# DRSY/EasyKV

Hardware: AMD Instinct MI355X
Metric: decode_tokens_per_sec (higher is better)
Workload: dtype f16 storage / f32 accumulate; 1 GPU; bench-D decode at fixed budget: B=1 L=32 Hq=32 H=32 D=128 budget=2048 T=2049 kv_policy=roco (Llama2-7B shape, budget=50% of S=4096); parallelism=1 GPU, layers_per_launch=32, layers_per_rank=32, sequences_per_launch=1, n_split=1, fused=True, slot_map=scattered (random permutation: long-run steady state), prewarm_steps=4096, hipgraph=False, overlap_scorer=False, handoff=False

## Files before the change

### easykv_amd/csrc/ekv_attn_decode.inc

```
#ifdef EKV_TAIL_PROFILE
#define EKV_STAMP(i) do { if (threadIdx.x == 0) stamps[i] = __builtin_readcyclecounter(); } while (0)
#endif
#include "ekv_decode_stream.h"
#include "ekv_decode_tail.h"
#ifndef EKV_KV8
#define EKV_KV8 0
#endif
#ifndef EKV_BATCH
#define EKV_BATCH 0
#endif
#if EKV_BATCH && EKV_KV8
#error "batch instances: 16-bit rows, plain keys"
#endif
#define ekv_attn_decode_kernel EKV_KERNEL_NAME(ekv_attn_decode_kernel)
#define ekv_decode_fused_kernel EKV_KERNEL_NAME(ekv_decode_fused_kernel)
#ifndef EKV_SPLIT_KU
#define EKV_SPLIT_KU (EKV_KV8 ? 4 : 8)
#endif
#ifndef EKV_FUSED_KU
#define EKV_FUSED_KU (EKV_KV8 ? 4 : 8)
#endif
#ifndef EKV_ROPE_KU
#define EKV_ROPE_KU(rep) ((rep) == 4 ? 8 : 4)
#endif

namespace {

constexpr int kEPL = EKV_KV8 ? 16 : 8;

template <int D, int REP, bool ROPE, bool SLOT_LDS>
__global__ void __launch_bounds__(256) ekv_attn_decode_kernel(const EkvAttnArgs EKV_ARG_A EKV_TB_PARAM) {
  EKV_SHADOW_A(blockIdx.z)
  using Gm = EkvDecodeGeom<D>;
  extern __shared__ __attribute__((aligned(16))) char smem[];
  int32_t* s_slot = reinterpret_cast<int32_t*>(smem);
  float* s_part = reinterpret_cast<float*>(smem + (SLOT_LDS ? ekv_align((size_t)a.rows_per_split * 4, 16) : 0));

  const int split = blockIdx.x % a.n_split, qgrp = blockIdx.x / a.n_split, h = blockIdx.y, ll = blockIdx.z;
  const int rep_all = a.n_q_heads / a.n_kv_heads;
  const int hq0 = h * rep_all + qgrp * REP;
  const int nrep = (REP == 1 || REP == 2) ? REP : min(REP, rep_all - qgrp * REP);
  const int tid = threadIdx.x;
  const int t0 = split * a.rows_per_split;
  const int t1 = min(a.n_slots, t0 + a.rows_per_split);
  const size_t head_row = ((size_t)(a.layer_begin + ll) * a.n_kv_heads + h) * a.cap;
  if (SLOT_LDS) {
    for (int i = tid; i < t1 - t0; i += 256) s_slot[i] = a.slot_of_pos[head_row + t0 + i];
    __syncthreads();
  }

  float m[REP], l[REP], o[REP][kEPL];
  float* logits = a.logits ? a.logits + ((size_t)ll * a.n_q_heads + hq0) * a.t_pad : nullptr;
  constexpr int KU = (!ROPE && !SLOT_LDS && REP <= 2) ? EKV_SPLIT_KU : (EKV_KV8 ? 4 : 8);
  ekv_decode_stream<D, REP, ROPE, SLOT_LDS, 4, false, KU>(a, SLOT_LDS ? s_slot : a.slot_of_pos + head_row, logits, a.t_pad, t0, t1,
                                                          ll, h, head_row, m, l, o, nullptr, EkvNoop(), nrep, hq0);

  ekv_decode_wave_combine<D, REP>(m, l, o);
  ekv_decode_stash<D, REP>(s_part, m, l, o);
  __syncthreads();
  const bool fold_here = a.arrive != nullptr;
  for (int idx = tid; idx < REP * D; idx += 256) {
    const int r = idx / D, d = idx % D;
    if (r >= nrep) continue;
    float mm, ls, os;
    ekv_decode_reduce<D, REP>(s_part, r, d, mm, ls, os);
    float* dst = a.partials + (((size_t)ll * a.n_q_heads + hq0 + r) * a.n_split + split) * Gm::PS;
    if (fold_here) {
      if (d == 0) {
        ekv_store_sc1(dst, mm);
        ekv_store_sc1(dst + 1, ls);
      }
      ekv_store_sc1(dst + 2 + d, os);
    } else {
      if (d == 0) {
        dst[0] = mm;
        dst[1] = ls;
      }
      dst[2 + d] = os;
    }
  }
  if (!fold_here) return;
  asm volatile("s_waitcnt vmcnt(0)" ::: "memory");
  __syncthreads();
  uint32_t* s_last = reinterpret_cast<uint32_t*>(s_part);
  if (tid == 0) {
    uint32_t* word = a.arrive + (size_t)EKV_ARRIVE_ROW(ll) * a.n_kv_heads + h;
    const uint32_t old = __hip_atomic_fetch_add(word, 1u, __ATOMIC_RELAXED, __HIP_MEMORY_SCOPE_AGENT);
    const bool last = (int)(old + 1u) == a.n_split;
    if (last) __hip_atomic_store(word, 0u, __ATOMIC_RELAXED, __HIP_MEMORY_SCOPE_AGENT);
    *s_last = last ? 1u : 0u;
  }
  __syncthreads();
  if (*s_last == 0u) return;
  const __amdgpu_buffer_rsrc_t rsrc = __builtin_amdgcn_make_buffer_rsrc(
      a.partials + (size_t)ll * a.n_q_heads * a.n_split * Gm::PS, 0, (int)((size_t)a.n_q_heads * a.n_split * Gm::PS * 4), 0x00020000);
  for (int idx = tid; idx < nrep * D; idx += 256) {
    const int r = idx / D, d = idx % D;
    const size_t row = (size_t)ll * a.n_q_heads + hq0 + r;
    a.out_direct[row * D + d] = ekv_to_e(ekv_fold_partials_buf_auto(rsrc, (unsigned)((hq0 + r) * a.n_split * Gm::PS), a.n_split, Gm::PS, d));
  }
}

template <int D, int REP, bool ROPE, int ITEMS, int NW, bool SLOT>
__global__ void __launch_bounds__(64 * NW, (NW >= 8 ? (REP == 1 ? 2 : 1) : (SLOT && ITEMS > 12 ? 2 : (REP == 1 ? 4 : (REP == 2 ? 3 : 2))))) ekv_decode_fused_kernel(const EkvAttnArgs EKV_ARG_A, const EkvScoreArgs EKV_ARG_SC EKV_TB_PARAM) {
  EKV_SHADOW_A(blockIdx.z)
  EKV_SHADOW_SC(blockIdx.z)
  using Gm = EkvDecodeGeom<D, NW>;
  extern __shared__ __attribute__((aligned(16))) char smem[];
  const int h = blockIdx.y, ll = blockIdx.z, tid = threadIdx.x;
  const int lane = tid & 63, wave = tid >> 6;
  const int T = a.n_slots;
  const int nrep = (REP == 1 || REP == 2) ? REP : a.n_q_heads / a.n_kv_heads;
  const bool roco = sc.policy == EKV_POLICY_ROCO;
  const bool scored = roco || sc.policy == EKV_POLICY_H2O_HEAD || sc.policy == EKV_POLICY_TOVA;
  const int off = scored ? sc.score_off : 0;
  const int W = SLOT ? a.phys_extent : T - off;
  const int w_pad = (int)ekv_align((size_t)W, 256);
#ifdef EKV_NO_PHYS
  constexpr bool PHYS = false;
#else
  constexpr bool PHYS = !ROPE;
#endif
  const int l_pad = a.l_pad;
  float* s_logit = reinterpret_cast<float*>(smem);
  float* s_part = s_logit + (size_t)REP * l_pad;
  float* sS = s_part + (size_t)Gm::NP * REP * Gm::PS + ((Gm::NP * REP * Gm::PS) & 3 ? 4 - ((Gm::NP * REP * Gm::PS) & 3) : 0);
  float* sQ = sS + w_pad;
  float* sC = sQ + w_pad;
  RedN<NW> red;
  red.buf = reinterpret_cast<unsigned long long*>(sS + (size_t)(roco ? (SLOT ? 2 : 3) : 1) * w_pad);
  red.phase = 0;
  red.lane = lane;
  red.wave = wave;
  const size_t head_row = ((size_t)(a.layer_begin + ll) * a.n_kv_heads + h) * a.cap;
#ifdef EKV_TAIL_PROFILE
  unsigned long long* stamps = reinterpret_cast<unsigned long long*>(sc.tova_row) + ((size_t)ll * a.n_kv_heads + h) * 8;
#endif
  EKV_STAMP(0);
  constexpr bool kOrders = D == 128 && REP == 1 && !ROPE && NW == 4 && SLOT && ITEMS <= 12 && !EKV_KV8 && !EKV_BATCH;
  bool order_k = false;
  if constexpr (kOrders) {
    const int om = a.fused_order & 3;
    if (om == 2) {
      order_k = scored;
    } else if (om == 1 && scored) {
      uint32_t* s_flag = reinterpret_cast<uint32_t*>(red.buf);
      if (tid == 0) {
        const uint32_t hw = __builtin_amdgcn_s_getreg(63492);
        const int src = (a.fused_order >> 4) & 3;
        const uint32_t x = src == 0 ? (hw >> 16) & 15u : (src == 1 ? hw & 15u : (uint32_t)(ll * a.n_kv_heads + h));
        const bool below = (x & ((a.fused_order >> 8) & 15u)) < ((a.fused_order >> 12) & 15u);
        *s_flag = below != (((a.fused_order >> 6) & 1) != 0) ? 1u : 0u;
      }
      __syncthreads();
      order_k = __builtin_amdgcn_readfirstlane((int)*s_flag) != 0;
    }
  }
  const int32_t* slot_row = a.slot_of_pos + head_row;
  uint32_t* s_deadw = reinterpret_cast<uint32_t*>(red.buf + 2 * NW * 8);
  if (scored) ekv_tail_prefetch_rows<NW, false>(sc, head_row, W, w_pad, roco, sS, sQ, sC, !SLOT);
  float g_old = 0.f, c_new = 0.f;
  int nb = 0;
  if (SLOT) {
    const size_t head = (size_t)(a.layer_begin + ll) * a.n_kv_heads + h;
    g_old = sc.slot_state[4 * head];
    nb = reinterpret_cast<const int32_t*>(sc.slot_state)[4 * head + 1];
    c_new = sc.cnt_tail[head_row + T - 1] - g_old;
  }
  const int E = a.phys_extent;
  const int fl_idx = T - 1 + tid;
  int fl = 0;
  if (PHYS) {
    fl = slot_row[min(fl_idx, a.cap - 1)];
    const int n_words = (int)ekv_align((size_t)E, 128) / 32;
    for (int i = tid; i < n_words; i += 64 * NW)
      s_deadw[i] = i * 32 >= E ? ~0u : (i * 32 + 32 > E ? ~0u << (E & 31) : 0u);
  }
  auto mask_ready = [&]() {
    ekv_lds_barrier();
    if (fl_idx < a.cap && fl < E) atomicOr(&s_deadw[fl >> 5], 1u << (fl & 31));
    for (int i = fl_idx + 64 * NW; i < a.cap; i += 64 * NW) {
      const int row = slot_row[i];
      if (row < E) atomicOr(&s_deadw[row >> 5], 1u << (row & 31));
    }
    ekv_lds_barrier();
  };

  if constexpr (kOrders) {
    if (order_k) {
      constexpr int LPR = Gm::LPR;
      const int sub = lane % LPR, grp = lane / LPR;
      const int new_row = slot_row[T - 1];
      const uint8_t* s_dead = reinterpret_cast<const uint8_t*>(s_deadw);
      const uint4 qv = reinterpret_cast<const uint4*>(a.q + ((size_t)ll * a.n_q_heads + h) * D)[sub];
      float mk = EKV_NEG_INF;
      ekv_decode_plane_loop<D, NW>(a.k, head_row, E, mask_ready, [&](uint4 (&kr)[8], const int j0) {
        const unsigned dead8 = (unsigned)s_dead[j0 >> 3];
        float s[8];
#pragma unroll
        for (int u = 0; u < 8; ++u) {
          const float acc = ekv_group_sum<LPR>(ekv_dot8(qv, kr[u], 0.f));
          s[u] = !((dead8 >> u) & 1u) ? acc / a.sm_div : EKV_NEG_INF;
        }
        float mine = s[0];
#pragma unroll
        for (int u = 1; u < 8; ++u) mine = (sub == u) ? s[u] : mine;
        if (sub < 8 && !((dead8 >> sub) & 1u)) s_logit[j0 + sub] = mine;
#pragma unroll
        for (int u = 0; u < 8; ++u) mk = fmaxf(mk, s[u]);
      });
      const __half* v_new_row = a.v_new + ((size_t)ll * a.n_kv_heads + h) * D;
      if (wave == 0 && grp == 0) {
        const uint4 kn = reinterpret_cast<const uint4*>(a.k_new + ((size_t)ll * a.n_kv_heads + h) * D)[sub];
        const uint4 vn = reinterpret_cast<const uint4*>(v_new_row)[sub];
        const size_t off_new = (head_row + new_row) * D;
        reinterpret_cast<uint4*>(a.k_w + off_new)[sub] = kn;
        reinterpret_cast<uint4*>(a.v_w + off_new)[sub] = vn;
        const float acc = ekv_group_sum<LPR>(ekv_dot8(qv, kn, 0.f)) / a.sm_div;
        if (sub == 0) s_logit[new_row] = acc;
        mk = fmaxf(mk, acc);
      }
      ekv_tail_prefetch_ragged<NW>(sc, head_row, W, roco, sS, sQ, sC, false);
      float cC[ITEMS];
      int32_t cB[ITEMS];
#pragma unroll
      for (int it = 0; it < ITEMS; ++it) {
        const int j = min(tid + it * 64 * NW, a.cap - 1);
        cC[it] = roco ? sc.score_cnt[head_row + j] : 0.f;
        cB[it] = sc.birth[head_row + j];
      }
      EKV_STAMP(1);
      mk = ekv_wave_max(mk);
      if (lane == 0) s_part[(size_t)wave * Gm::PS] = mk;
      __syncthreads();
      uint32_t* s_hist = s_deadw + ekv_align(ekv_align((size_t)l_pad, 128) / 32, 4);
      ekv_decode_tail_slot<REP, ITEMS, NW, true>(sc, ll, h, head_row, T, E, s_logit, l_pad, sS, sQ, cC, cB, red, s_hist,
                                                 reinterpret_cast<unsigned long long*>(s_part), Gm::NP * REP * Gm::PS / 2, s_part, Gm::NP,
                                                 Gm::PS, s_deadw, new_row, g_old, c_new, nb, nrep);
      EKV_STAMP(2);
      float m[1] = {EKV_NEG_INF}, l[1] = {0.f}, o[1][8];
#pragma unroll
      for (int i = 0; i < 8; ++i) o[0][i] = 0.f;
      ekv_decode_plane_loop<D, NW>(a.v, head_row, E, EkvNoop(), [&](uint4 (&vr)[8], const int j0) {
        const unsigned dead8 = (unsigned)s_dead[j0 >> 3];
        float s[8];
        if (dead8 == 0xFFu) {
#pragma unroll
          for (int u = 0; u < 8; ++u) s[u] = EKV_NEG_INF;
        } else {
          const float4 s0 = *reinterpret_cast<const float4*>(s_logit + j0), s1 = *reinterpret_cast<const float4*>(s_logit + j0 + 4);
          s[0] = s0.x, s[1] = s0.y, s[2] = s0.z, s[3] = s0.w, s[4] = s1.x, s[5] = s1.y, s[6] = s1.z, s[7] = s1.w;
        }
        if (dead8 != 0u) {
#pragma unroll
          for (int u = 0; u < 8; ++u)
            if ((dead8 >> u) & 1u) {
              vr[u] = uint4{0, 0, 0, 0};
              s[u] = EKV_NEG_INF;
            }
        }
        float mx = s[0];
#pragma unroll
        for (int u = 1; u < 8; ++u) mx = fmaxf(mx, s[u]);
        const float mn = fmaxf(m[0], mx);
        if (mn == EKV_NEG_INF) return;
        const float alpha = exp2f((m[0] - mn) * EKV_LOG2E);
        l[0] *= alpha;
#pragma unroll
        for (int i = 0; i < 8; ++i) o[0][i] *= alpha;
#pragma unroll
        for (int u = 0; u < 8; ++u) {
          const float p = exp2f((s[u] - mn) * EKV_LOG2E);
          l[0] += p;
          ekv_axpy8(p, vr[u], o[0]);
        }
        m[0] = mn;
      });
      if (wave == 0 && grp == 0) {
        const uint4 vn = reinterpret_cast<const uint4*>(v_new_row)[sub];
        const float acc = s_logit[new_row];
        const float mn = fmaxf(m[0], acc);
        const float alpha = m[0] == EKV_NEG_INF ? 0.f : exp2f((m[0] - mn) * EKV_LOG2E);
        const float p = exp2f((acc - mn) * EKV_LOG2E);
        l[0] = l[0] * alpha + p;
#pragma unroll
        for (int i = 0; i < 8; ++i) o[0][i] *= alpha;
        ekv_axpy8(p, vn, o[0]);
        m[0] = mn;
      }
      ekv_decode_wave_combine<D, 1>(m, l, o);
      ekv_decode_stash<D, 1, NW>(s_part, m, l, o);
      __syncthreads();
      for (int d = tid; d < D; d += 64 * NW) {
        float mm, ls, os;
        ekv_decode_reduce<D, 1, NW>(s_part, 0, d, mm, ls, os);
        sc.out[((size_t)ll * a.n_q_heads + h) * D + d] = ekv_to_e(os / ls);
      }
      EKV_STAMP(5);
#ifdef EKV_TAIL_PROFILE
      if (tid == 0) {
        stamps[3] = 1;
        stamps[6] = __builtin_amdgcn_s_getreg(63492);
        stamps[7] = __builtin_amdgcn_s_getreg(63508);
      }
#endif
      return;
    }
  }

  constexpr int KUF = ROPE ? EKV_ROPE_KU(REP) : EKV_FUSED_KU;
  float m[REP], l[REP], o[REP][kEPL];
  if (PHYS)
    ekv_decode_stream<D, REP, ROPE, false, NW, PHYS, KUF>(a, slot_row, s_logit, l_pad, 0, T, ll, h, head_row, m, l, o,
                                                     reinterpret_cast<const uint8_t*>(s_deadw), mask_ready, nrep, h * nrep);
  else
    ekv_decode_stream<D, REP, ROPE, false, NW, false, KUF>(a, slot_row, s_logit, l_pad, 0, T, ll, h, head_row, m, l, o, nullptr, EkvNoop(),
                                                      nrep, h * nrep);
  if (scored) ekv_tail_prefetch_ragged<NW>(sc, head_row, W, roco, sS, sQ, sC, !SLOT);
  float cC[SLOT ? ITEMS : 1];
  int32_t cB[SLOT ? ITEMS : 1];
  if (SLOT) {
#pragma unroll
    for (int it = 0; it < (SLOT ? ITEMS : 1); ++it) {
      const int j = min(tid + it * 64 * NW, a.cap - 1);
      cC[it] = roco ? sc.score_cnt[head_row + j] : 0.f;
      cB[it] = sc.birth[head_row + j];
    }
  }

  EKV_STAMP(1);
  ekv_decode_wave_combine<D, REP>(m, l, o);
  ekv_decode_stash<D, REP, NW>(s_part, m, l, o);
  __syncthreads();
  for (int idx = tid; idx < nrep * D; idx += 64 * NW) {
    const int r = idx / D, d = idx % D;
    float mm, ls, os;
    ekv_decode_reduce<D, REP, NW>(s_part, r, d, mm, ls, os);
    sc.out[((size_t)ll * a.n_q_heads + h * nrep + r) * D + d] = ekv_to_e(os / ls);
  }

  uint32_t* s_hist = s_deadw + ekv_align(ekv_align((size_t)l_pad, 128) / 32, 4);
  if constexpr (SLOT) {
    ekv_decode_tail_slot<REP, ITEMS, NW>(sc, ll, h, head_row, T, E, s_logit, l_pad, sS, sQ, cC, cB, red, s_hist,
                                         reinterpret_cast<unsigned long long*>(s_part), Gm::NP * REP * Gm::PS / 2, s_part, Gm::NP, Gm::PS,
                                         s_deadw, slot_row[T - 1], g_old, c_new, nb, nrep);
  } else {
    ekv_decode_tail<REP, ITEMS, NW, PHYS>(sc, ll, h, head_row, T, off, W, s_logit, l_pad, sS, sQ, sC, red, s_hist,
                                          reinterpret_cast<unsigned long long*>(s_part), Gm::NP * REP * Gm::PS / 2, s_part, Gm::NP, Gm::PS, nrep);
  }
  EKV_STAMP(5);
#ifdef EKV_TAIL_PROFILE
  if (tid == 0) {
    stamps[6] = __builtin_amdgcn_s_getreg(63492);
    stamps[7] = __builtin_amdgcn_s_getreg(63508);
  }
#endif
}

template <int REP>
hipError_t launch(const EkvAttnArgs& a EKV_TB_DECL, int layer_count, hipStream_t s) {
  using Gm = EkvDecodeGeom<EKV_D>;
  const size_t part = (size_t)Gm::NP * REP * Gm::PS * 4;
  const int rep_all = a.n_q_heads / a.n_kv_heads;
  const dim3 grid(a.n_split * ((rep_all + REP - 1) / REP), a.n_kv_heads, layer_count);
  if ((a.cap & 3) == 0 && a.cap >= 16) {
    hipLaunchKernelGGL((ekv_attn_decode_kernel<EKV_D, REP, EKV_ROPE, false>), grid, dim3(256), part, s, a EKV_TB_PASS);
  } else {
    const size_t lds = ekv_align((size_t)a.rows_per_split * 4, 16) + part;
    if (lds > 48 * 1024)
      (void)hipFuncSetAttribute(reinterpret_cast<const void*>(&ekv_attn_decode_kernel<EKV_D, REP, EKV_ROPE, true>),
                                hipFuncAttributeMaxDynamicSharedMemorySize, (int)lds);
    hipLaunchKernelGGL((ekv_attn_decode_kernel<EKV_D, REP, EKV_ROPE, true>), grid, dim3(256), lds, s, a EKV_TB_PASS);
  }
  return hipGetLastError();
}

template <int REP, int NW = 8>
size_t fused_lds(int t_pad, int l_pad, int n_state) { return ekv_fused_lds<EKV_D, REP, NW>(t_pad, l_pad, n_state); }

template <int REP, int ITEMS, int NW, bool SLOT>
hipError_t launch_fused_k(const EkvAttnArgs& a, const EkvScoreArgs& sc EKV_TB_DECL, int layer_count, hipStream_t s) {
  const size_t lds = SLOT ? fused_lds<REP, NW>(a.phys_extent, a.l_pad, sc.policy == EKV_POLICY_ROCO ? 2 : 1)
                          : fused_lds<REP, NW>(a.t_pad, a.l_pad, sc.policy == EKV_POLICY_ROCO ? 3 : 1);
  if (lds > 48 * 1024)
    (void)hipFuncSetAttribute(reinterpret_cast<const void*>(&ekv_decode_fused_kernel<EKV_D, REP, EKV_ROPE, ITEMS, NW, SLOT>),
                              hipFuncAttributeMaxDynamicSharedMemorySize, (int)lds);
  hipLaunchKernelGGL((ekv_decode_fused_kernel<EKV_D, REP, EKV_ROPE, ITEMS, NW, SLOT>), dim3(1, a.n_kv_heads, layer_count),
                     dim3(64 * NW), lds, s, a, sc EKV_TB_PASS);
  return hipGetLastError();
}

template <int REP, int NW>
hipError_t launch_fused_nw(const EkvAttnArgs& a, const EkvScoreArgs& sc EKV_TB_DECL, int layer_count, hipStream_t s) {
  constexpr int NT = 64 * NW, I0 = (2304 + NT - 1) / NT, I1 = (6144 + NT - 1) / NT;
  if (sc.birth != nullptr) {
    if constexpr (!EKV_ROPE && !EKV_BATCH && REP <= 4) {
      if (a.phys_extent <= NT * I0) return launch_fused_k<REP, I0, NW, true>(a, sc EKV_TB_PASS, layer_count, s);
      if (a.phys_extent <= NT * I1) return launch_fused_k<REP, I1, NW, true>(a, sc EKV_TB_PASS, layer_count, s);
    }
    return hipErrorInvalidValue;
  }
  if (a.n_slots <= NT * I0) return launch_fused_k<REP, I0, NW, false>(a, sc EKV_TB_PASS, layer_count, s);
  return launch_fused_k<REP, I1, NW, false>(a, sc EKV_TB_PASS, layer_count, s);
}
template <int REP>
hipError_t launch_fused(const EkvAttnArgs& a, const EkvScoreArgs& sc EKV_TB_DECL, int layer_count, int nw, hipStream_t s) {
  return nw == 8 ? launch_fused_nw<REP, 8>(a, sc EKV_TB_PASS, layer_count, s) : launch_fused_nw<REP, 4>(a, sc EKV_TB_PASS, layer_count, s);
}

}

#if EKV_ROPE
#define EKV_KEYS rope
#else
#define EKV_KEYS plain
#endif
#define EKV_SYM(fn) EKV_FN_DECODE(fn, EKV_D, EKV_KEYS, EKV_ELEM, EKV_ROWS, EKV_BATCHING)

hipError_t EKV_SYM(ekv_launch_attn_decode)(const EkvAttnArgs& a, const EkvSeqTable* tb, int rep, int layer_count, hipStream_t s) {
  if (rep < 1) return hipErrorInvalidValue;
  switch (rep) {
    case 1: return launch<1>(a EKV_TB_DEREF, layer_count, s);
    case 2: return launch<2>(a EKV_TB_DEREF, layer_count, s);
    case 3: case 4: return launch<4>(a EKV_TB_DEREF, layer_count, s);
    default: return launch<8>(a EKV_TB_DEREF, layer_count, s);
  }
}

hipError_t EKV_SYM(ekv_launch_decode_fused)(const EkvAttnArgs& a, const EkvScoreArgs& sc, const EkvSeqTable* tb, int rep, int layer_count,
                                            int nw, hipStream_t s) {
  switch (rep) {
    case 1: return launch_fused<1>(a, sc EKV_TB_DEREF, layer_count, nw, s);
    case 2: return launch_fused<2>(a, sc EKV_TB_DEREF, layer_count, nw, s);
    case 3: case 4: return launch_fused<4>(a, sc EKV_TB_DEREF, layer_count, nw, s);
    case 5: case 6: case 7: case 8: return launch_fused<8>(a, sc EKV_TB_DEREF, layer_count, nw, s);
    default: return hipErrorInvalidValue;
  }
}
```

### easykv_amd/csrc/ekv_decode_stream.h

```cpp
#pragma once
#include "ekv_common.h"
#include "ekv_kernels.h"

constexpr int kU = 8;

template <int D, int NW = 4, int KU = kU, int EPL = 8>
struct EkvDecodeGeom {
  static constexpr int LIVE = D / EPL;
  static constexpr int LPR = LIVE <= 4 ? 4 : (LIVE <= 8 ? 8 : 16);
  static constexpr int G = 64 / LPR;
  static constexpr int RW = G * KU;
  static constexpr int NP = NW;
  static constexpr int PS = D + 2;
};

template <int D, int REP, int NW = 8>
inline size_t ekv_fused_lds(int t_pad, int l_pad, int n_state) {
  using Gm = EkvDecodeGeom<D, NW>;
  const size_t part = ekv_align((size_t)Gm::NP * REP * Gm::PS, 4);
  return ((size_t)REP * l_pad + part + (size_t)n_state * ekv_align((size_t)t_pad, 256)) * 4 + 2 * NW * 8 * 8 +
         ekv_align(ekv_align((size_t)l_pad, 128) / 8, 16) + 264 * 4;
}
template <int D>
inline size_t ekv_fused_lds_max(int rep, int t_pad, int l_pad, int nw) {
  switch (rep) {
    case 1: return nw == 8 ? ekv_fused_lds<D, 1, 8>(t_pad, l_pad, 3) : ekv_fused_lds<D, 1, 4>(t_pad, l_pad, 3);
    case 2: return nw == 8 ? ekv_fused_lds<D, 2, 8>(t_pad, l_pad, 3) : ekv_fused_lds<D, 2, 4>(t_pad, l_pad, 3);
    case 3: case 4: return nw == 8 ? ekv_fused_lds<D, 4, 8>(t_pad, l_pad, 3) : ekv_fused_lds<D, 4, 4>(t_pad, l_pad, 3);
    default: return nw == 8 ? ekv_fused_lds<D, 8, 8>(t_pad, l_pad, 3) : ekv_fused_lds<D, 8, 4>(t_pad, l_pad, 3);
  }
}

struct EkvNoop {
  __device__ __forceinline__ void operator()() const {}
};
#ifndef EKV_ROPE_MOCK
#define EKV_ROPE_MOCK 0
#endif
template <int D, int REP, bool ROPE, bool SLOT_LDS, int NW = 4, bool PHYS = false, int KU = kU, typename MaskReady = EkvNoop, int EPL = 8>
__device__ __forceinline__ void ekv_decode_stream(const EkvAttnArgs& a, const int32_t* s_slot, float* logit_out,
                                                  int logit_stride, int t0, int t1_in, int ll, int h, size_t head_row,
                                                  float (&m)[REP], float (&l)[REP], float (&o)[REP][EPL],
                                                  const uint8_t* s_dead = nullptr, MaskReady mask_ready = MaskReady(),
                                                  int n_rep_real = 0, int q_head0 = -1) {
  using Gm = EkvDecodeGeom<D, NW, KU, EPL>;
  constexpr int LPR = Gm::LPR, RW = Gm::RW, LIVE = Gm::LIVE;
  constexpr bool KV8 = EPL == 16;
  static_assert(EPL == 8 || (KV8 && !ROPE && LIVE == LPR), "FP8 rows: plain keys, head_dim 64 / 128");
  constexpr int ESZ = KV8 ? 1 : 2;
  constexpr bool PADDED = LIVE != LPR;
  constexpr int kNW = NW;
  static_assert(!(PHYS && (ROPE || SLOT_LDS)), "physical-order streaming: plain keys, global slot map");
  static_assert((KU == 4 || KU == 8 || KU == 16) && (!PHYS || KU <= 8), "4, 8 or 16 rows per lane group; the dead-row mask is one byte per 8 rows");
  const int tid = threadIdx.x, lane = tid & 63, wave = tid >> 6;
  const int sub = lane % LPR, grp = lane / LPR;
  const int t_new = a.n_slots - 1;
  int t1 = t1_in;
  const bool live_lane = !PADDED || sub < LIVE;
  const int nrep = n_rep_real > 0 ? n_rep_real : REP;
  const int hq0 = q_head0 >= 0 ? q_head0 : h * REP;

  uint4 qv[REP], qv1[REP];
  float qf[REP][8];
#pragma unroll
  for (int r = 0; r < REP; ++r) {
    const __half* qp = a.q + ((size_t)ll * a.n_q_heads + hq0 + min(r, nrep - 1)) * D;
    qv[r] = live_lane ? reinterpret_cast<const uint4*>(qp)[sub * (EPL / 8)] : uint4{0, 0, 0, 0};
    qv1[r] = KV8 ? reinterpret_cast<const uint4*>(qp)[sub * 2 + 1] : uint4{0, 0, 0, 0};
#pragma unroll
    for (int i = 0; i < 8; ++i) qf[r][i] = 0.f;
    if (ROPE && live_lane) {
      const int half_d = D / 2;
      const float* c = a.rope_cos + (size_t)t_new * D;
      const float* s = a.rope_sin + (size_t)t_new * D;
#pragma unroll
      for (int i = 0; i < 8; ++i) {
        const int d = sub * 8 + i;
        const int dp = d < half_d ? d + half_d : d - half_d;
        const float x = __half2float(qp[d]), y = __half2float(qp[dp]);
        qf[r][i] = x * c[d] + (d < half_d ? -y : y) * s[d];
      }
    }
  }

#ifndef EKV_ROPE_EXACT
#define EKV_ROPE_EXACT 0
#endif
  constexpr bool kRopeExact = EKV_ROPE_EXACT || REP == 8;
  const float sgn = (sub < LIVE / 2) ? -1.f : 1.f;
  const int tab_off = (sub % (LIVE / 2)) * 8;
  auto rope_seed = [&](int j, ekv_f2 (&cc)[4], ekv_f2 (&ss)[4]) {
#if EKV_ROPE_MOCK == 1
    float one = 1.f, zero = 0.25f;
    asm volatile("" : "+v"(one), "+v"(zero));
#pragma unroll
    for (int i = 0; i < 4; ++i) cc[i] = ekv_f2{one, one}, ss[i] = ekv_f2{zero, zero};
    (void)j;
#else
    const float4* c4 = reinterpret_cast<const float4*>(a.rope_cos + (size_t)j * D + tab_off);
    const float4* s4 = reinterpret_cast<const float4*>(a.rope_sin + (size_t)j * D + tab_off);
    const float4 c0 = c4[0], c1 = c4[1], s0 = s4[0], s1 = s4[1];
    cc[0] = ekv_f2{c0.x, c0.y}, cc[1] = ekv_f2{c0.z, c0.w}, cc[2] = ekv_f2{c1.x, c1.y}, cc[3] = ekv_f2{c1.z, c1.w};
    ss[0] = ekv_f2{s0.x, s0.y} * sgn, ss[1] = ekv_f2{s0.z, s0.w} * sgn, ss[2] = ekv_f2{s1.x, s1.y} * sgn, ss[3] = ekv_f2{s1.z, s1.w} * sgn;
#endif
  };
  ekv_f2 stp_c[4], stp_s[4];
  if (ROPE && !kRopeExact) rope_seed(min(1, a.n_slots - 1), stp_c, stp_s);
  auto rope_advance = [&](ekv_f2 (&cc)[4], ekv_f2 (&ss)[4]) {
#pragma unroll
    for (int i = 0; i < 4; ++i) {
      const ekv_f2 cn = __builtin_elementwise_fma(cc[i], stp_c[i], -(ss[i] * stp_s[i]));
      ss[i] = __builtin_elementwise_fma(ss[i], stp_c[i], cc[i] * stp_s[i]);
      cc[i] = cn;
    }
  };
  auto rope_rotate = [&](const uint4& kv, const ekv_f2 (&cc)[4], const ekv_f2 (&ss)[4], float (&kp)[8]) {
    uint4 other;
#if EKV_ROPE_MOCK == 2
    other = kv;
#else
    if (PADDED) {
      const int src = (lane & ~(LPR - 1)) | (sub < LIVE / 2 ? sub + LIVE / 2 : (sub < LIVE ? sub - LIVE / 2 : sub));
      other.x = __shfl(kv.x, src, 64);
      other.y = __shfl(kv.y, src, 64);
      other.z = __shfl(kv.z, src, 64);
      other.w = __shfl(kv.w, src, 64);
    } else {
      other.x = __shfl_xor(kv.x, LPR / 2, 64);
      other.y = __shfl_xor(kv.y, LPR / 2, 64);
      other.z = __shfl_xor(kv.z, LPR / 2, 64);
      other.w = __shfl_xor(kv.w, LPR / 2, 64);
    }
#endif
    const ekv_h8 kh = __builtin_bit_cast(ekv_h8, kv), oh = __builtin_bit_cast(ekv_h8, other);
#pragma unroll
    for (int i = 0; i < 4; ++i) {
      const ekv_f2 k2 = {(float)kh[2 * i], (float)kh[2 * i + 1]}, o2 = {(float)oh[2 * i], (float)oh[2 * i + 1]};
      const ekv_f2 r2 = __builtin_elementwise_fma(k2, cc[i], o2 * ss[i]);
      kp[2 * i] = r2[0];
      kp[2 * i + 1] = r2[1];
    }
  };

  const __half* k_new_row = a.k_new + ((size_t)ll * a.n_kv_heads + h) * D;
  const __half* v_new_row = a.v_new + ((size_t)ll * a.n_kv_heads + h) * D;
  const int slot_base = SLOT_LDS ? t0 : 0;
#pragma unroll
  for (int r = 0; r < REP; ++r) {
    m[r] = EKV_NEG_INF;
    l[r] = 0.f;
#pragma unroll
    for (int i = 0; i < EPL; ++i) o[r][i] = 0.f;
  }

  const bool has_new = t_new >= t0 && t_new < t1;
  if (has_new) t1 = t_new;
  auto appended_row = [&]() {
    if (!(has_new && wave == 0 && grp == 0)) return;
    const int slot_new = s_slot[t_new - slot_base];
    uint4 kn = uint4{0, 0, 0, 0}, vn = uint4{0, 0, 0, 0};
    const size_t off = (head_row + slot_new) * D;
    float ksn = 1.f, vsn = 1.f;
    if constexpr (KV8) {
      float kf[16], vf[16];
      const uint4* kq = reinterpret_cast<const uint4*>(k_new_row) + sub * 2;
      const uint4* vq = reinterpret_cast<const uint4*>(v_new_row) + sub * 2;
      float ka = fmaxf(ekv_widen8_amax(kq[0], kf), ekv_widen8_amax(kq[1], kf + 8));
      float va = fmaxf(ekv_widen8_amax(vq[0], vf), ekv_widen8_amax(vq[1], vf + 8));
      ksn = ekv_fp8_row_scale(ekv_group_max<LPR>(ka));
      vsn = ekv_fp8_row_scale(ekv_group_max<LPR>(va));
      kn = uint4{ekv_fp8_quant4(kf[0], kf[1], kf[2], kf[3], ksn), ekv_fp8_quant4(kf[4], kf[5], kf[6], kf[7], ksn),
                 ekv_fp8_quant4(kf[8], kf[9], kf[10], kf[11], ksn), ekv_fp8_quant4(kf[12], kf[13], kf[14], kf[15], ksn)};
      vn = uint4{ekv_fp8_quant4(vf[0], vf[1], vf[2], vf[3], vsn), ekv_fp8_quant4(vf[4], vf[5], vf[6], vf[7], vsn),
                 ekv_fp8_quant4(vf[8], vf[9], vf[10], vf[11], vsn), ekv_fp8_quant4(vf[12], vf[13], vf[14], vf[15], vsn)};
      reinterpret_cast<uint4*>(reinterpret_cast<uint8_t*>(a.k_w) + off)[sub] = kn;
      reinterpret_cast<uint4*>(reinterpret_cast<uint8_t*>(a.v_w) + off)[sub] = vn;
      if (sub == 0) {
        a.k_scale[head_row + slot_new] = ksn;
        a.v_scale[head_row + slot_new] = vsn;
      }
    } else if (live_lane) {
      kn = reinterpret_cast<const uint4*>(k_new_row)[sub];
      vn = reinterpret_cast<const uint4*>(v_new_row)[sub];
      reinterpret_cast<uint4*>(a.k_w + off)[sub] = kn;
      reinterpret_cast<uint4*>(a.v_w + off)[sub] = vn;
    }
    float kpn[8];
    if (ROPE) {
      ekv_f2 cn[4], sn[4];
      rope_seed(t_new, cn, sn);
      rope_rotate(kn, cn, sn, kpn);
    }
#pragma unroll
    for (int r = 0; r < REP; ++r) {
      float acc;
      if (ROPE) {
        acc = 0.f;
#pragma unroll
        for (int i = 0; i < 8; ++i) acc = fmaf(kpn[i], qf[r][i], acc);
      } else if constexpr (KV8) {
        acc = ekv_dot16_fp8(qv[r], qv1[r], kn, 0.f);
      } else {
        acc = ekv_dot8(qv[r], kn, 0.f);
      }
      acc = KV8 ? ekv_group_sum<LPR>(acc) * ksn / a.sm_div : ekv_group_sum<LPR>(acc) / a.sm_div;
      if (logit_out != nullptr && sub == 0 && r < nrep) logit_out[(size_t)r * logit_stride + (PHYS ? slot_new : t_new)] = acc;
      const float mn = fmaxf(m[r], acc);
      const float alpha = m[r] == EKV_NEG_INF ? 0.f : exp2f((m[r] - mn) * EKV_LOG2E);
      const float p = exp2f((acc - mn) * EKV_LOG2E);
      l[r] = l[r] * alpha + p;
#pragma unroll
      for (int i = 0; i < EPL; ++i) o[r][i] *= alpha;
      if constexpr (KV8) ekv_axpy16_fp8(p * vsn, vn, o[r]);
      else ekv_axpy8(p, vn, o[r]);
      m[r] = mn;
    }
  };
  if (!PHYS && t1 <= t0) {
    appended_row();
    return;
  }

  if (PHYS) t1 = a.phys_extent;
  const int last_slot = PHYS ? 0 : s_slot[t1 - 1 - slot_base];
  const int idx_cap = (a.cap - KU) & ~(KU - 1);
  uint4 iv[KU / 4];
#pragma unroll
  for (int i = 0; i < KU / 4; ++i) iv[i] = uint4{0, 0, 0, 0};
  if (!PHYS && !SLOT_LDS && t0 + wave * RW < t1) {
    const uint4* ip = reinterpret_cast<const uint4*>(s_slot + min(t0 + wave * RW + grp * KU, idx_cap));
#pragma unroll
    for (int i = 0; i < KU / 4; ++i) iv[i] = ip[i];
  }
  auto iteration = [&](const int base, auto&& after_issue) {
    uint4 kr[KU], vr[KU];
    float ksc[KV8 ? KU : 1], vsc[KV8 ? KU : 1];
    const int j0 = base + grp * KU;
    if constexpr (KV8 && PHYS) {
      if (j0 + KU <= a.cap) {
        const float4* k4 = reinterpret_cast<const float4*>(a.k_scale + head_row + j0);
        const float4* v4 = reinterpret_cast<const float4*>(a.v_scale + head_row + j0);
#pragma unroll
        for (int i = 0; i < KU / 4; ++i) {
          const float4 kk = k4[i], vv = v4[i];
          ksc[4 * i] = kk.x, ksc[4 * i + 1] = kk.y, ksc[4 * i + 2] = kk.z, ksc[4 * i + 3] = kk.w;
          vsc[4 * i] = vv.x, vsc[4 * i + 1] = vv.y, vsc[4 * i + 2] = vv.z, vsc[4 * i + 3] = vv.w;
        }
      } else {
#pragma unroll
        for (int u = 0; u < KU; ++u) {
          ksc[u] = a.k_scale[head_row + min(j0 + u, a.cap - 1)];
          vsc[u] = a.v_scale[head_row + min(j0 + u, a.cap - 1)];
        }
      }
    }
    int cur[KU];
#pragma unroll
    for (int i = 0; i < KU / 4; ++i) {
      cur[4 * i] = (int)iv[i].x;
      cur[4 * i + 1] = (int)iv[i].y;
      cur[4 * i + 2] = (int)iv[i].z;
      cur[4 * i + 3] = (int)iv[i].w;
    }
    if (!PHYS && !SLOT_LDS && base + kNW * RW < t1) {
      const uint4* ip = reinterpret_cast<const uint4*>(s_slot + min(j0 + kNW * RW, idx_cap));
#pragma unroll
      for (int i = 0; i < KU / 4; ++i) iv[i] = ip[i];
    }
#pragma unroll
    for (int u = 0; u < KU; ++u) {
      const int j = j0 + u;
      const int jj = j < t1 ? j : t1 - 1;
      const int row = PHYS ? jj : (SLOT_LDS ? s_slot[jj - t0] : (j < t1 ? cur[u] : last_slot));
      const char* kp = reinterpret_cast<const char*>(a.k) + (head_row + row) * (D * ESZ);
      const char* vp = reinterpret_cast<const char*>(a.v) + (head_row + row) * (D * ESZ);
      if constexpr (KV8 && !PHYS) {
        ksc[u] = a.k_scale[head_row + row];
        vsc[u] = a.v_scale[head_row + row];
      }
      if (live_lane) {
        kr[u] = __builtin_bit_cast(uint4, __builtin_nontemporal_load(reinterpret_cast<const ekv_u4*>(kp) + sub));
        vr[u] = __builtin_bit_cast(uint4, __builtin_nontemporal_load(reinterpret_cast<const ekv_u4*>(vp) + sub));
      } else {
        kr[u] = vr[u] = uint4{0, 0, 0, 0};
      }
    }
    ekv_f2 rc[4], rs[4];
    if (ROPE) rope_seed(min(j0, t1 - 1), rc, rs);
    after_issue();
    const unsigned dead8 = PHYS ? (KU == 4 ? ((unsigned)s_dead[j0 >> 3] >> (j0 & 4)) & 0xFu : (unsigned)s_dead[j0 >> 3]) : 0u;
    if (PHYS && dead8 != 0u) {
#pragma unroll
      for (int u = 0; u < KU; ++u)
        if ((dead8 >> u) & 1u) {
          vr[u] = uint4{0, 0, 0, 0};
          if constexpr (KV8) vsc[u] = 0.f;
        }
    }
    float sall[ROPE ? REP : 1][KU];
    if (ROPE) {
#pragma unroll
      for (int u = 0; u < KU; ++u) {
        float kp[8];
        rope_rotate(kr[u], rc, rs, kp);
        if (u + 1 < KU) {
          if (kRopeExact) rope_seed(min(j0 + u + 1, t1 - 1), rc, rs);
          else rope_advance(rc, rs);
        }
#pragma unroll
        for (int r = 0; r < REP; ++r) {
          float acc = 0.f;
#pragma unroll
          for (int i = 0; i < 8; ++i) acc = fmaf(kp[i], qf[r][i], acc);
          acc = ekv_group_sum<LPR>(acc);
          sall[r][u] = (j0 + u < t1) ? acc / a.sm_div : EKV_NEG_INF;
        }
      }
    }
#pragma unroll
    for (int r = 0; r < REP; ++r) {
      float s[KU];
#pragma unroll
      for (int u = 0; u < KU; ++u) {
        if (ROPE) {
          s[u] = sall[r][u];
        } else {
          float acc = KV8 ? ekv_dot16_fp8(qv[r], qv1[r], kr[u], 0.f) : ekv_dot8(qv[r], kr[u], 0.f);
          acc = ekv_group_sum<LPR>(acc);
          if constexpr (KV8) acc *= ksc[u];
          s[u] = (PHYS ? !((dead8 >> u) & 1u) : (j0 + u < t1)) ? acc / a.sm_div : EKV_NEG_INF;
        }
      }
      constexpr int NST = (KU + LPR - 1) / LPR;
#pragma unroll
      for (int st = 0; st < NST; ++st) {
        const int mu = sub + st * LPR;
        float mine = s[0];
#pragma unroll
        for (int u = 1; u < KU; ++u) mine = (mu == u) ? s[u] : mine;
        if (logit_out != nullptr && mu < KU && r < nrep && (PHYS ? !((dead8 >> mu) & 1u) : (j0 + mu < t1)))
          logit_out[(size_t)r * logit_stride + j0 + mu] = mine;
      }
      float mx = s[0];
#pragma unroll
      for (int u = 1; u < KU; ++u) mx = fmaxf(mx, s[u]);
      const float mn = fmaxf(m[r], mx);
      if (mn == EKV_NEG_INF) continue;
      const float alpha = exp2f((m[r] - mn) * EKV_LOG2E);
      l[r] *= alpha;
#pragma unroll
      for (int i = 0; i < EPL; ++i) o[r][i] *= alpha;
#pragma unroll
      for (int u = 0; u < KU; ++u) {
        const float p = exp2f((s[u] - mn) * EKV_LOG2E);
        l[r] += p;
        if constexpr (KV8) ekv_axpy16_fp8(p * vsc[u], vr[u], o[r]);
        else ekv_axpy8(p, vr[u], o[r]);
      }
      m[r] = mn;
    }
  };
  int base = t0 + wave * RW;
  if (PHYS) {
    if (t1 > (kNW - 1) * RW) {
      iteration(base, mask_ready);
      base += kNW * RW;
    } else {
      mask_ready();
    }
  }
  for (; base < t1; base += kNW * RW) iteration(base, EkvNoop());
  appended_row();
}

template <int D, int REP, int EPL = 8>
__device__ __forceinline__ void ekv_decode_wave_combine(float (&m)[REP], float (&l)[REP], float (&o)[REP][EPL]) {
  using Gm = EkvDecodeGeom<D, 4, kU, EPL>;
#pragma unroll
  for (int off = Gm::LPR; off < 64; off <<= 1) {
#pragma unroll
    for (int r = 0; r < REP; ++r) {
      const float mo = __shfl_xor(m[r], off, 64), lo = __shfl_xor(l[r], off, 64);
      const float mn = fmaxf(m[r], mo);
      const float wa = (m[r] == EKV_NEG_INF) ? 0.f : exp2f((m[r] - mn) * EKV_LOG2E);
      const float wb = (mo == EKV_NEG_INF) ? 0.f : exp2f((mo - mn) * EKV_LOG2E);
      l[r] = l[r] * wa + lo * wb;
#pragma unroll
      for (int i = 0; i < EPL; ++i) o[r][i] = o[r][i] * wa + __shfl_xor(o[r][i], off, 64) * wb;
      m[r] = mn;
    }
  }
}

template <int D, int REP, int NW = 4, int EPL = 8>
__device__ __forceinline__ void ekv_decode_stash(float* s_part, const float (&m)[REP], const float (&l)[REP],
                                                 const float (&o)[REP][EPL]) {
  using Gm = EkvDecodeGeom<D, NW, kU, EPL>;
  const int lane = threadIdx.x & 63, wave = threadIdx.x >> 6;
  const int sub = lane % Gm::LPR, grp = lane / Gm::LPR;
  if (grp != 0 || sub >= Gm::LIVE) return;
#pragma unroll
  for (int r = 0; r < REP; ++r) {
    float* p = s_part + ((size_t)wave * REP + r) * Gm::PS;
    if (sub == 0) {
      p[0] = m[r];
      p[1] = l[r];
    }
#pragma unroll
    for (int i = 0; i < EPL; ++i) p[2 + sub * EPL + i] = o[r][i];
  }
}

template <int D, int REP, int NW = 4>
__device__ __forceinline__ void ekv_decode_reduce(const float* s_part, int r, int d, float& mm, float& ls, float& os) {
  using Gm = EkvDecodeGeom<D, NW>;
  mm = EKV_NEG_INF;
#pragma unroll
  for (int i = 0; i < Gm::NP; ++i) mm = fmaxf(mm, s_part[((size_t)i * REP + r) * Gm::PS]);
  ls = 0.f;
  os = 0.f;
#pragma unroll
  for (int i = 0; i < Gm::NP; ++i) {
    const float* p = s_part + ((size_t)i * REP + r) * Gm::PS;
    const float w = (p[0] == EKV_NEG_INF) ? 0.f : exp2f((p[0] - mm) * EKV_LOG2E);
    ls += p[1] * w;
    os += p[2 + d] * w;
  }
}

template <int D, int NW, typename First, typename Consume>
__device__ __forceinline__ void ekv_decode_plane_loop(const __half* plane, size_t head_row, int t1, First&& first, Consume&& consume) {
  using Gm = EkvDecodeGeom<D, NW, 8, 8>;
  static_assert(Gm::LIVE == Gm::LPR, "whole lane groups");
  constexpr int RW = Gm::RW, STEP = NW * RW;
  const int lane = threadIdx.x & 63, wave = threadIdx.x >> 6;
  const int sub = lane % Gm::LPR, grp = lane / Gm::LPR;
  auto request = [&](uint4 (&r)[8], int base) {
    const int j0 = base + grp * 8;
#pragma unroll
    for (int u = 0; u < 8; ++u) {
      const int row = j0 + u < t1 ? j0 + u : t1 - 1;
      const char* p = reinterpret_cast<const char*>(plane) + (head_row + row) * (D * 2);
      r[u] = __builtin_bit_cast(uint4, __builtin_nontemporal_load(reinterpret_cast<const ekv_u4*>(p) + sub));
    }
  };
  uint4 ra[8], rb[8];
  int base = wave * RW;
  request(ra, base);
  first();
  while (base < t1) {
    request(rb, base + STEP);
    consume(ra, base + grp * 8);
    base += STEP;
    if (base >= t1) break;
    request(ra, base + STEP);
    consume(rb, base + grp * 8);
    base += STEP;
  }
}
```

Measured before the change: 5544 tokens/s.

## Stream V plane through a per-row load ring in fused decode

Adds a ring-buffered plane loader that keeps R rows of loads in flight per lane group. Each row's load is reissued as soon as that row is consumed, instead of double-buffering whole 8-row batches. The V pass of the fused decode kernel now uses this ring (default depth 16), and an optional K-pass version stays disabled by default. The aim is steadier memory-level parallelism and less stall time between batches, at the cost of more registers held for the ring and reworked softmax bookkeeping split across group and row callbacks.

```diff
diff --git a/easykv_amd/csrc/ekv_attn_decode.inc b/easykv_amd/csrc/ekv_attn_decode.inc
--- a/easykv_amd/csrc/ekv_attn_decode.inc
+++ b/easykv_amd/csrc/ekv_attn_decode.inc
@@ -22,6 +22,12 @@
 #endif
 #ifndef EKV_ROPE_KU
 #define EKV_ROPE_KU(rep) ((rep) == 4 ? 8 : 4)
+#endif
+#ifndef EKV_VRING_R
+#define EKV_VRING_R 16
+#endif
+#ifndef EKV_KRING_R
+#define EKV_KRING_R 0
 #endif
 
 namespace {
@@ -194,6 +200,20 @@
       const uint8_t* s_dead = reinterpret_cast<const uint8_t*>(s_deadw);
       const uint4 qv = reinterpret_cast<const uint4*>(a.q + ((size_t)ll * a.n_q_heads + h) * D)[sub];
       float mk = EKV_NEG_INF;
+#if EKV_KRING_R
+      unsigned dead_k = 0u;
+      int jk = 0;
+      ekv_decode_plane_ring<D, NW, EKV_KRING_R>(a.k, head_row, E, mask_ready, [&](const int j0) {
+        dead_k = (unsigned)s_dead[j0 >> 3];
+        jk = j0;
+      }, [&](const int u, const uint4& kr) {
+        const float acc = ekv_group_sum<LPR>(ekv_dot8(qv, kr, 0.f));
+        const bool dead = (dead_k >> u) & 1u;
+        const float s = !dead ? acc / a.sm_div : EKV_NEG_INF;
+        if (sub == u && !dead) s_logit[jk + u] = s;
+        mk = fmaxf(mk, s);
+      });
+#else
       ekv_decode_plane_loop<D, NW>(a.k, head_row, E, mask_ready, [&](uint4 (&kr)[8], const int j0) {
         const unsigned dead8 = (unsigned)s_dead[j0 >> 3];
         float s[8];
@@ -209,6 +229,7 @@
 #pragma unroll
         for (int u = 0; u < 8; ++u) mk = fmaxf(mk, s[u]);
       });
+#endif
       const __half* v_new_row = a.v_new + ((size_t)ll * a.n_kv_heads + h) * D;
       if (wave == 0 && grp == 0) {
         const uint4 kn = reinterpret_cast<const uint4*>(a.k_new + ((size_t)ll * a.n_kv_heads + h) * D)[sub];
@@ -241,6 +262,46 @@
       float m[1] = {EKV_NEG_INF}, l[1] = {0.f}, o[1][8];
 #pragma unroll
       for (int i = 0; i < 8; ++i) o[0][i] = 0.f;
+#if EKV_VRING_R
+      float s[8], mn = EKV_NEG_INF;
+      unsigned dead_v = 0u;
+      bool live = false;
+      ekv_decode_plane_ring<D, NW, EKV_VRING_R>(a.v, head_row, E, EkvNoop(), [&](const int j0) {
+        dead_v = (unsigned)s_dead[j0 >> 3];
+        if (dead_v == 0xFFu) {
+#pragma unroll
+          for (int u = 0; u < 8; ++u) s[u] = EKV_NEG_INF;
+        } else {
+          const float4 s0 = *reinterpret_cast<const float4*>(s_logit + j0), s1 = *reinterpret_cast<const float4*>(s_logit + j0 + 4);
+          s[0] = s0.x, s[1] = s0.y, s[2] = s0.z, s[3] = s0.w, s[4] = s1.x, s[5] = s1.y, s[6] = s1.z, s[7] = s1.w;
+        }
+        if (dead_v != 0u) {
+#pragma unroll
+          for (int u = 0; u < 8; ++u)
+            if ((dead_v >> u) & 1u) s[u] = EKV_NEG_INF;
+        }
+        float mx = s[0];
+#pragma unroll
+        for (int u = 1; u < 8; ++u) mx = fmaxf(mx, s[u]);
+        mn = fmaxf(m[0], mx);
+        live = mn != EKV_NEG_INF;
+        if (!live) return;
+        const float alpha = exp2f((m[0] - mn) * EKV_LOG2E);
+        l[0] *= alpha;
+#pragma unroll
+        for (int i = 0; i < 8; ++i) o[0][i] *= alpha;
+        m[0] = mn;
+      }, [&](const int u, const uint4& vr) {
+        if (!live) return;
+        uint4 v = vr;
+        if (dead_v != 0u) {
+          if ((dead_v >> u) & 1u) v = uint4{0, 0, 0, 0};
+        }
+        const float p = exp2f((s[u] - mn) * EKV_LOG2E);
+        l[0] += p;
+        ekv_axpy8(p, v, o[0]);
+      });
+#else
       ekv_decode_plane_loop<D, NW>(a.v, head_row, E, EkvNoop(), [&](uint4 (&vr)[8], const int j0) {
         const unsigned dead8 = (unsigned)s_dead[j0 >> 3];
         float s[8];
@@ -276,6 +337,7 @@
         }
         m[0] = mn;
       });
+#endif
       if (wave == 0 && grp == 0) {
         const uint4 vn = reinterpret_cast<const uint4*>(v_new_row)[sub];
         const float acc = s_logit[new_row];
diff --git a/easykv_amd/csrc/ekv_decode_stream.h b/easykv_amd/csrc/ekv_decode_stream.h
--- a/easykv_amd/csrc/ekv_decode_stream.h
+++ b/easykv_amd/csrc/ekv_decode_stream.h
@@ -458,3 +458,37 @@
     base += STEP;
   }
 }
+
+template <int D, int NW, int R, typename First, typename Group, typename Row>
+__device__ __forceinline__ void ekv_decode_plane_ring(const __half* plane, size_t head_row, int t1, First&& first, Group&& group, Row&& row) {
+  using Gm = EkvDecodeGeom<D, NW, 8, 8>;
+  static_assert(Gm::LIVE == Gm::LPR, "whole lane groups");
+  static_assert(R == 16 || R == 20 || R == 24, "ring depths tried: 16, 20, 24 rows per lane group");
+  constexpr int RW = Gm::RW, STEP = NW * RW;
+  constexpr int P = R % 8 == 0 ? R : 2 * R;
+  const int lane = threadIdx.x & 63, wave = __builtin_amdgcn_readfirstlane((int)(threadIdx.x >> 6));
+  const int sub = lane % Gm::LPR, grp = lane / Gm::LPR;
+  const char* head_p = reinterpret_cast<const char*>(plane) + head_row * (D * 2);
+  const uint32_t lane_off = sub * 16, last_off = (uint32_t)(t1 - 1) * (D * 2) + lane_off;
+  auto request = [&](uint4& r, int j) {
+    const uint32_t off = min((uint32_t)j * (D * 2) + lane_off, last_off);
+    r = __builtin_bit_cast(uint4, __builtin_nontemporal_load(reinterpret_cast<const ekv_u4*>(head_p + off)));
+  };
+  uint4 ring[R];
+  int gb = wave * (RW / 8) + grp;
+#pragma unroll
+  for (int i = 0; i < R; ++i) request(ring[i], (gb + (i / 8) * (STEP / 8)) * 8 + i % 8);
+  first();
+  int left = wave * RW < t1 ? (t1 - wave * RW + STEP - 1) / STEP : 0;
+  for (; left > 0; left -= P / 8, gb += (P / 8) * (STEP / 8)) {
+#pragma unroll
+    for (int i = 0; i < P; ++i) {
+      if (i % 8 == 0) {
+        if (i / 8 >= left) break;
+        group((gb + (i / 8) * (STEP / 8)) * 8);
+      }
+      row(i % 8, ring[i % R]);
+      request(ring[i % R], (gb + ((i + R) / 8) * (STEP / 8)) * 8 + (i + R) % 8);
+    }
+  }
+}
```

Measured after the change: 5449 tokens/s. 0.983x the previous value.
